# cvjena/semantic-embeddings

Measured on AMD Instinct MI355X. Metric: retrieval_Mpairs_per_sec, higher is better.
Workload: dtype f32

## Files before the change

semantic-embeddings_amd/csrc/rank_rows.hip:

```cpp
#include "se_common.h"
#include <stdlib.h>
#include <atomic>
#include <type_traits>

namespace se {

constexpr int RK_THREADS = 512;
constexpr int RK_WAVES = RK_THREADS / WAVE;
constexpr int RK_ITEMS = 16;
constexpr int RK_TILE = RK_THREADS * RK_ITEMS;
constexpr int RK_WCHUNK = RK_TILE / RK_WAVES;
constexpr int RK_NB = 256;

struct RankLds {
    uint32_t gbase[4][RK_NB];
    uint32_t wcnt[RK_WAVES][RK_NB];
    uint32_t tile_start[RK_NB];
    uint32_t wave_tot[RK_WAVES];
    uint32_t tkeys[RK_TILE];
    uint32_t tidx[RK_TILE];
};

__device__ __forceinline__ uint32_t wave_excl_scan(uint32_t v, uint32_t &total)
{
// ... 11 lines not shown
    RankLds &L = *reinterpret_cast<RankLds *>(rk_raw);
    const int tid = threadIdx.x, lane = tid & 63, wave = tid >> 6;
    const uint64_t lt_mask = (lane == 0) ? 0ull : (~0ull >> (64 - lane));

    uint32_t *kA = ws + (int64_t)blockIdx.x * 4 * n_pad;
    uint32_t *iA = kA + n_pad, *kB = iA + n_pad, *iB = kB + n_pad;
    const int ntiles = (N + RK_TILE - 1) / RK_TILE;

    for (int64_t row = blockIdx.x; row < Q; row += gridDim.x) {
        const float *drow = pdist + row * ldp;

        wg_barrier();
        for (int i = tid; i < 4 * RK_NB; i += RK_THREADS) (&L.gbase[0][0])[i] = 0;
        wg_barrier();
        for (int i = tid; i < N; i += RK_THREADS) {
            const uint32_t key = canon_key(drow[i]);
            atomicAdd(&L.gbase[0][key & 0xFF], 1u);
            atomicAdd(&L.gbase[1][(key >> 8) & 0xFF], 1u);
            atomicAdd(&L.gbase[2][(key >> 16) & 0xFF], 1u);
            atomicAdd(&L.gbase[3][key >> 24], 1u);
        }
        wg_barrier();
        if (wave < 4) {
            uint32_t c[4], s = 0;
#pragma unroll
            for (int j = 0; j < 4; j++) { c[j] = L.gbase[wave][lane * 4 + j]; s += c[j]; }
            uint32_t tot;
            uint32_t run = wave_excl_scan(s, tot);
#pragma unroll
            for (int j = 0; j < 4; j++) { L.gbase[wave][lane * 4 + j] = run; run += c[j]; }
        }
        wg_barrier();

#pragma unroll 1
        for (int p = 0; p < 4; p++) {
            const int shift = p * 8;
            const uint32_t *sk = (p & 1) ? kA : kB;
            const uint32_t *si = (p & 1) ? iA : iB;
            uint32_t *dk = (p & 1) ? kB : kA;
            uint32_t *di = (p & 1) ? iB : iA;
            const bool last = (p == 3);
#pragma unroll 1
            for (int t = 0; t < ntiles; t++) {
                const int tbase = t * RK_TILE;
                const int tcount = (N - tbase < RK_TILE) ? (N - tbase) : RK_TILE;
                const int wbeg = wave * RK_WCHUNK;

                uint32_t key[RK_ITEMS], idx[RK_ITEMS];
                if (p == 0) {
#pragma unroll
                    for (int s = 0; s < RK_ITEMS; s++) {
                        const int li = wbeg + s * WAVE + lane;
                        const int gi = tbase + li;
                        const float f = drow[gi < N ? gi : N - 1];
                        key[s] = (li < tcount) ? canon_key(f) : 0xFFFFFFFFu;
                        idx[s] = (uint32_t)gi;
                    }
                } else {
#pragma unroll
                    for (int s = 0; s < RK_ITEMS; s++) {
                        const int li = wbeg + s * WAVE + lane;
                        const int gi = tbase + li;
                        const int gc = gi < N ? gi : N - 1;
                        const uint32_t k = sk[gc], i2 = si[gc];
                        key[s] = (li < tcount) ? k : 0xFFFFFFFFu;
                        idx[s] = i2;
                    }
                }
#pragma unroll
                for (int j = 0; j < RK_NB / WAVE; j++) L.wcnt[wave][j * WAVE + lane] = 0;
#pragma unroll
                for (int s = 0; s < RK_ITEMS; s++) {
                    const int li = wbeg + s * WAVE + lane;
                    if (li < tcount) atomicAdd(&L.wcnt[wave][(key[s] >> shift) & 0xFF], 1u);
                }
                wg_barrier();
                uint32_t my_total = 0;
                if (tid < RK_NB) {
                    uint32_t run = 0;
#pragma unroll
                    for (int w = 0; w < RK_WAVES; w++) {
                        const uint32_t c = L.wcnt[w][tid];
                        L.wcnt[w][tid] = run;
                        run += c;
                    }
                    my_total = run;
                    uint32_t wtot;
                    const uint32_t ex = wave_excl_scan(my_total, wtot);
                    if (lane == 63) L.wave_tot[wave] = wtot;
                    L.tile_start[tid] = ex;
                }
                wg_barrier();
                if (tid < RK_NB) {
                    uint32_t add = 0;
                    for (int w = 0; w < wave; w++) add += L.wave_tot[w];
                    const uint32_t st = L.tile_start[tid] + add;
                    L.tile_start[tid] = st;
#pragma unroll
                    for (int w = 0; w < RK_WAVES; w++) L.wcnt[w][tid] += st;
                }
                wg_barrier();

                volatile uint32_t *cur = L.wcnt[wave];
#pragma unroll
                for (int s = 0; s < RK_ITEMS; s++) {
                    const int li = wbeg + s * WAVE + lane;
                    const bool valid = li < tcount;
                    const uint32_t dgt = (key[s] >> shift) & 0xFF;
                    uint64_t peers = __ballot(valid);
#pragma unroll
                    for (int bb = 0; bb < 8; bb++) {
                        const bool bit = (dgt >> bb) & 1u;
                        const uint64_t m = __ballot(bit && valid);
                        peers &= bit ? m : ~m;
                    }
                    if (valid) {
                        const int rnk = __popcll(peers & lt_mask);
                        const int npeers = __popcll(peers);
                        const uint32_t base = cur[dgt];
                        if (rnk == npeers - 1) cur[dgt] = base + (uint32_t)npeers;
                        L.tkeys[base + rnk] = key[s];
                        L.tidx[base + rnk] = idx[s];
                    }
                }
                wg_barrier();

#pragma unroll
                for (int j = 0; j < RK_ITEMS; j++) {
                    const int i = j * RK_THREADS + tid;
                    if (i < tcount) {
                        const uint32_t k = L.tkeys[i];
                        const uint32_t id = L.tidx[i];
                        const uint32_t d = (k >> shift) & 0xFF;
                        const uint32_t gpos = L.gbase[p][d] + ((uint32_t)i - L.tile_start[d]);
                        if (last) {
                            if (IDX64) ((int64_t *)rank)[row * ldr + gpos] = (int64_t)id;
                            else ((int32_t *)rank)[row * ldr + gpos] = (int32_t)id;
                        } else {
                            dk[gpos] = k;
                            di[gpos] = id;
                        }
                    }
                }
                wg_barrier();
                if (tid < RK_NB) L.gbase[p][tid] += my_total;
            }
        }
    }
}


constexpr int RR_THREADS = 512;
constexpr int RR_WAVES = RR_THREADS / WAVE;
constexpr int RR_SCAN_THREADS = 512;
constexpr int RR_SCAN_WAVES = RR_SCAN_THREADS / WAVE;
static_assert((53248 + RR_THREADS - 1) / RR_THREADS <= 104, "rows of up to 53,248 columns: 104 keys per thread");
constexpr int RR_G = 8;
constexpr int RR_MAX_N = 53248;

__device__ __forceinline__ void differ_mask(uint32_t d, uint32_t &lo, uint32_t &hi)
{
    lo = 0;
    hi = 0;
#pragma unroll
    for (int bb = 0; bb < 8; bb += 2) {
        uint32_t s0 = (uint32_t)__builtin_amdgcn_sbfe((int)d, bb, 1);
        uint32_t s1 = (uint32_t)__builtin_amdgcn_sbfe((int)d, bb + 1, 1);
        asm volatile("" : "+v"(s0), "+v"(s1));
        const uint64_t m0 = __ballot(s0 != 0), m1 = __ballot(s1 != 0);
        lo = __builtin_amdgcn_bitop3_b32(lo, (uint32_t)m0, s0, 0xF6);
        hi = __builtin_amdgcn_bitop3_b32(hi, (uint32_t)(m0 >> 32), s0, 0xF6);
        lo = __builtin_amdgcn_bitop3_b32(lo, (uint32_t)m1, s1, 0xF6);
        hi = __builtin_amdgcn_bitop3_b32(hi, (uint32_t)(m1 >> 32), s1, 0xF6);
    }
}

constexpr uint32_t RR_KEY_NAN = 0xFF900000u;
__device__ __forceinline__ uint32_t rr_pad_key(uint32_t lane) { return 0xFFA00000u + ((lane % 6u) << 20) + (lane << 11) + lane; }
__device__ __forceinline__ uint32_t rr_key(uint32_t u, bool pad, uint32_t pad_key)
{
    const uint32_t sx = (uint32_t)((int32_t)u >> 31);
    uint32_t k = __builtin_amdgcn_bitop3_b32(u, sx, 0x80000000u, 0x1E);
    k -= sx;
    const float f = __uint_as_float(u);
    k = (f != f) ? RR_KEY_NAN : k;
    return pad ? pad_key : k;
}

__device__ __forceinline__ int32_t rr_clamp_i32(int32_t x, int32_t lo, int32_t hi) { return min(max(x, lo), hi); }

template <typename T>
__device__ __forceinline__ void opaque(T &x) { asm volatile("" : "+v"(x)); }

__device__ __forceinline__ uint32_t lds_off(const void *p) { return (uint32_t)(uintptr_t)p; }
__device__ __forceinline__ void lds_wait() { asm volatile("s_waitcnt lgkmcnt(0)" ::: "memory"); }
__device__ __forceinline__ void lds_st16_lo(uint32_t addr, uint32_t v) { asm volatile("ds_write_b16 %0, %1" ::"v"(addr), "v"(v) : "memory"); }
__device__ __forceinline__ void lds_st16_hi(uint32_t addr, uint32_t v) { asm volatile("ds_write_b16_d16_hi %0, %1" ::"v"(addr), "v"(v) : "memory"); }
__device__ __forceinline__ uint32_t rr_dst_mad(uint32_t ir, uint32_t xb)
{
    uint32_t a;
    asm("v_mad_u32_u16 %0, %1, 2, %2" : "=v"(a) : "v"(ir), "s"(xb));
    return a;
}
template <int OFF>
__device__ __forceinline__ void lds_ld16(uint32_t &dst, uint32_t addr) { asm volatile("ds_read_u16 %0, %1 offset:%2" : "=v"(dst) : "v"(addr), "n"(OFF) : "memory"); }
template <int OFF>
__device__ __forceinline__ void lds_ld16x4_tr(uint64_t &dst, uint32_t addr) { asm volatile("ds_read_b64_tr_b16 %0, %1 offset:%2" : "=v"(dst) : "v"(addr), "n"(OFF) : "memory"); }
template <int K, typename T>
__device__ __forceinline__ void lds_wait_le(T &landed) { asm volatile("s_waitcnt lgkmcnt(%1)" : "+v"(landed) : "n"(K) : "memory"); }

constexpr int RR_RING = 12;
__host__ __device__ constexpr uint32_t rr_tr_lane_off(uint32_t lane) { return 128u * ((lane >> 2) & 3u) + 32u * (lane >> 4) + 8u * (lane & 3u); }
template <int ITEMS, bool HI, int I = 0>
struct RRRead {
    static constexpr int NT = ITEMS / 4, OPS = NT + ITEMS % 4, D = RR_RING / 2 - 1;
    static constexpr uint32_t SEL_LO16 = HI ? 0x05040100u : 0x03020504u;
    static constexpr uint32_t SEL_HI16 = HI ? 0x07060100u : 0x03020706u;
    static __device__ __forceinline__ void run(uint32_t (&a)[ITEMS], uint64_t (&t)[RR_RING / 2], uint32_t (&u)[4], uint32_t rt, uint32_t rb)
    {
        if constexpr (I < NT) lds_ld16x4_tr<I * 4 * WAVE * 2>(t[I % (RR_RING / 2)], rt);
        else if constexpr (I < OPS) lds_ld16<(3 * NT + I) * WAVE * 2>(u[I - NT], rb);
        if constexpr (I >= D) {
            constexpr int J = I - D;
            constexpr int newest = (I < OPS ? I : OPS - 1);
            if constexpr (J < NT) {
                uint64_t &v = t[J % (RR_RING / 2)];
                lds_wait_le<newest - J>(v);
                const uint32_t lo = (uint32_t)v, hi = (uint32_t)(v >> 32);
                a[4 * J + 0] = __builtin_amdgcn_perm(lo, a[4 * J + 0], SEL_LO16);
                a[4 * J + 1] = __builtin_amdgcn_perm(lo, a[4 * J + 1], SEL_HI16);
                a[4 * J + 2] = __builtin_amdgcn_perm(hi, a[4 * J + 2], SEL_LO16);
                a[4 * J + 3] = __builtin_amdgcn_perm(hi, a[4 * J + 3], SEL_HI16);
            } else {
                lds_wait_le<newest - J>(u[J - NT]);
                a[3 * NT + J] = __builtin_amdgcn_perm(u[J - NT], a[3 * NT + J], SEL_LO16);
            }
        }
        if constexpr (I + 1 < OPS + D) RRRead<ITEMS, HI, I + 1>::run(a, t, u, rt, rb);
    }
};
template <int ITEMS, bool HI>
__device__ __forceinline__ void rr_read_back(uint32_t (&a)[ITEMS], uint64_t (&ring)[RR_RING / 2], uint32_t rt, uint32_t rb)
{
    uint32_t u[4];
    RRRead<ITEMS, HI>::run(a, ring, u, rt, rb);
}

template <int ITEMS, int V, int S0, int I = 0>
struct RRRankFinish {
    static __device__ __forceinline__ void run(uint32_t (&ir)[ITEMS], uint32_t (&key)[ITEMS], uint32_t (&rnk)[V], uint32_t (&base)[V])
    {
        lds_wait_le<2 * (V - 1 - I) + 1>(base[I]);
        ir[S0 + I] = (ir[S0 + I] & 0xFFFF0000u) | (base[I] + rnk[I]);
        opaque(ir[S0 + I]);
        opaque(key[S0 + I]);
        if constexpr (I + 1 < V) RRRankFinish<ITEMS, V, S0, I + 1>::run(ir, key, rnk, base);
    }
};

template <int ITEMS, int S0 = 0>
struct RRRank {
    static __device__ __forceinline__ void run(uint32_t (&ir)[ITEMS], uint32_t (&key)[ITEMS], int shift, int lane, uint32_t cb)
    {
        constexpr int V = (ITEMS - S0 < RR_G) ? (ITEMS - S0) : RR_G;
        static_assert(2 * V - 1 <= 15, "lgkmcnt counts to 15");
        uint32_t rnk[V], base[V];
#pragma unroll
        for (int g = 0; g < V; g++) {
            const uint32_t d = (key[S0 + g] >> shift) & 0xFFu;
            uint32_t dlo, dhi;
            differ_mask(d, dlo, dhi);
            rnk[g] = (uint32_t)lane - wave_prefix_count(dlo, dhi);
            const uint32_t ca = cb + (d << 2);
            asm volatile("ds_read_b32 %0, %1" : "=v"(base[g]) : "v"(ca) : "memory");
            if (rnk[g] == 0) {
                const uint32_t np = 64u - (uint32_t)(__popc(dlo) + __popc(dhi));
                asm volatile("ds_add_u32 %0, %1" ::"v"(ca), "v"(np) : "memory");
            }
        }
        RRRankFinish<ITEMS, V, S0>::run(ir, key, rnk, base);
        __builtin_amdgcn_sched_barrier(0);
        if constexpr (S0 + V < ITEMS) RRRank<ITEMS, S0 + V>::run(ir, key, shift, lane, cb);
    }
};

typedef int rr_i32x4 __attribute__((ext_vector_type(4)));
typedef long long rr_i64x2 __attribute__((ext_vector_type(2)));
constexpr int RR_GH = 8;
constexpr int RR_HW_BITS = 11;
constexpr int RR_WIDE_WORDS = 2048;
constexpr uint32_t RR_TWO_SPAN = (1u << 24) - 3u;
constexpr int RR_TWO_OUT = 256;
constexpr int RR_IMG_RUN = 8;
constexpr int RR_IMG_WL = 3072;
constexpr int RR_IMG_MAX_ITEMS = 98;
constexpr uint32_t RR_IMG_NAN_PADHI = 0xFF0u;
constexpr int RR_IMG_SET_WORDS = 2048;
template <int ITEMS, bool PEEL, int S = 0>
struct RRRankHW {
    static __device__ __forceinline__ void run(uint32_t (&ir)[ITEMS], uint32_t (&key)[ITEMS], uint32_t (&r)[RR_GH], uint32_t (&sh)[RR_GH],
                                               uint32_t (&grp)[RR_GH], uint32_t shift, uint32_t hshift, uint32_t wlo, uint32_t whi, uint32_t cb,
                                               int lane, bool peel)
    {
        constexpr int SLOT = S % RR_GH;
        uint32_t ca = 0, inc = 0, shv = 0, g = 0xFFFFFFFFu;
        uint64_t part = ~0ull;
        if constexpr (S < ITEMS) {
            const uint32_t w = __builtin_amdgcn_ubfe(key[S], shift, wlo);
            const uint32_t h = __builtin_amdgcn_ubfe(key[S], hshift, whi);
            ca = cb + (w << 2);
            if constexpr (PEEL) {
                shv = h << 4;
                inc = 1u << shv;
            } else {
                inc = __umul24(h, 0xFFFFu) + 1u;
                shv = __umul24(h, 0x0202u) + 0x07060100u;
            }
            if constexpr (PEEL) {
                if (peel) {
                    const uint32_t d = w | (h << 11);
                    const bool in = (d == (uint32_t)__builtin_amdgcn_readfirstlane((int)d));
                    const uint64_t m = __ballot(in);
                    if (in) g = wave_prefix_count(m);
                    if (lane == 0) inc = (uint32_t)__popcll(m) << shv;
                    part = ~m | 1ull;
                }
            }
        }
        if constexpr (S >= RR_GH) {
            constexpr int J = S - RR_GH;
            constexpr int younger = ((S < ITEMS ? S : ITEMS) - 1) - J;
            lds_wait_le<younger>(r[SLOT]);
            if constexpr (PEEL) {
                const uint32_t lead = (uint32_t)__builtin_amdgcn_readfirstlane((int)r[SLOT]);
                const uint32_t own = (grp[SLOT] != 0xFFFFFFFFu) ? lead : r[SLOT];
                const uint32_t rank = __builtin_amdgcn_ubfe(own, sh[SLOT], 16u) + (grp[SLOT] != 0xFFFFFFFFu ? grp[SLOT] : 0u);
                ir[J] = (ir[J] & 0xFFFF0000u) | rank;
            } else {
                ir[J] = __builtin_amdgcn_perm(ir[J], r[SLOT], sh[SLOT]);
            }
            opaque(ir[J]);
            opaque(key[J]);
        }
        if constexpr (S < ITEMS) {
            sh[SLOT] = shv;
            grp[SLOT] = g;
            if constexpr (PEEL) {
                uint64_t saved;
                r[SLOT] = 0;
                asm volatile("s_and_saveexec_b64 %0, %4\n\tds_add_rtn_u32 %1, %2, %3\n\ts_mov_b64 exec, %0"
                             : "=&s"(saved), "+v"(r[SLOT])
                             : "v"(ca), "v"(inc), "s"(part)
                             : "memory");
            } else {
                asm volatile("ds_add_rtn_u32 %0, %1, %2" : "=v"(r[SLOT]) : "v"(ca), "v"(inc) : "memory");
            }
        }
        __builtin_amdgcn_sched_barrier(0);
        if constexpr (S + 1 < ITEMS + RR_GH) RRRankHW<ITEMS, PEEL, S + 1>::run(ir, key, r, sh, grp, shift, hshift, wlo, whi, cb, lane, peel);
    }
};

// ... 192 lines not shown
            }
            RR_T(8)
        }
        if constexpr (WIDE && VAR == 2) {
            uint32_t *stat = wave_tot;
            uint2 *outl = reinterpret_cast<uint2 *>(wcnt);
            const int n_row = row_len(row);
            int32_t mxi = 0;
            uint32_t umx = 0;
#pragma unroll
            for (int s = 0; s + 1 < ITEMS; s += 2) {
                mxi = max(max(mxi, rr_clamp_i32((int32_t)key[s], 0, 0x7F800000)), rr_clamp_i32((int32_t)key[s + 1], 0, 0x7F800000));
                umx = max(max(umx, key[s]), key[s + 1]);
            }
            if constexpr (ITEMS & 1) { mxi = max(mxi, rr_clamp_i32((int32_t)key[ITEMS - 1], 0, 0x7F800000)); umx = max(umx, key[ITEMS - 1]); }
            mxi = umx > 0xFF800000u ? 0x7F800000 : mxi;
#pragma unroll
            for (int off = 32; off > 0; off >>= 1) mxi = max(mxi, __shfl_xor(mxi, off, 64));
            if (lane == 0) stat[wave] = (uint32_t)mxi;
            if (tid == 0) stat[2 * RR_WAVES] = 0;
            RR_T(9)
            wg_barrier();
            RR_T(10)
#pragma unroll
            for (int w = 0; w < RR_WAVES; w++) mxi = max(mxi, (int32_t)stat[w]);
            const int32_t kmax = __builtin_amdgcn_readfirstlane(mxi);
            const int32_t lo = kmax > (int32_t)RR_TWO_SPAN ? kmax - (int32_t)RR_TWO_SPAN : 1, lo1 = lo - 1;
            uint32_t below_l = 0;
            {
                int wpos = wpos0;
                opaque(wpos);
#pragma unroll
                for (int s = 0; s < ITEMS; s++) below_l += ((int32_t)key[s] < lo) ? 1u : 0u;
                if (wave_s * (ITEMS * WAVE) + ITEMS * WAVE > n_row) {
                    int32_t lo_b = lo;
                    opaque(lo_b);
                    RR_PAD_LOOP(n_row, below_l -= (wpos + s * WAVE >= n_row && (int32_t)key[s] < lo_b) ? 1u : 0u;)
                }
            }
            uint32_t below_w = below_l;
#pragma unroll
            for (int off = 32; off > 0; off >>= 1) below_w += (uint32_t)__shfl_xor((int)below_w, off, 64);
            if (lane == 0) stat[RR_WAVES + wave] = below_w;
            RR_T(11)
            wg_barrier();
            uint32_t below = 0;
#pragma unroll
            for (int w = 0; w < RR_WAVES; w++) below += stat[RR_WAVES + w];
            two = kmax > 0 && below <= (uint32_t)RR_TWO_OUT;
            n_out = (int)below;
            if (two) {
                int wpos = wpos0;
                opaque(wpos);
                if (below_w != 0) {
                    int32_t lo_c = lo;
                    opaque(lo_c);
#pragma unroll
                    for (int s = 0; s < ITEMS; s++)
                        if ((int32_t)key[s] < lo_c && wpos + s * WAVE < n_row)
                            outl[atomicAdd(&stat[2 * RR_WAVES], 1u)] = make_uint2(rr_key(key[s], false, 0u), (uint32_t)(wpos + s * WAVE));
                }
#pragma unroll
                for (int s = 0; s < ITEMS; s++)
                    key[s] = (uint32_t)rr_clamp_i32(__builtin_elementwise_sub_sat((int32_t)key[s], lo1), 0, 0xFFFFFF) << 8;
                if (wave_s * (ITEMS * WAVE) + ITEMS * WAVE > n_row) {
                    RR_PAD_LOOP(n_row, key[s] = (wpos + s * WAVE >= n_row) ? 0xFFFFFF00u : key[s];)
                }
            } else {
                RR_CANON(n_row)
            }
            RR_T(8)
        }
        __builtin_amdgcn_sched_barrier(0);
        {
            int wpos = wpos0;
            opaque(wpos);
#pragma unroll
            for (int s = 0; s < ITEMS; s++) ir[s] = (uint32_t)(wpos + s * WAVE) << 16;
        }
#pragma unroll 1
        for (int p = 0; p < NPASS; p++) {
            const int shift = two ? 8 + 12 * p : (WIDE ? p * 10 : p * BITS);
            const int end = two ? (p == 1 ? 32 : 20)
                                : (WIDE ? (p == 2 ? 32 : shift + 10) : ((shift + BITS < 32) ? shift + BITS : 32));
            const bool wide = WIDE && (two || p == 2);
            uint32_t *pcnt = wcnt;
            int pcw = CNT_WORDS;
            const bool shared0 = IMG && two && p == 0;
            if (shared0) {
                pcnt = wlist;
                pcw = 0;
            } else if (wide) {
                if (!(RAWKEYS && two && p == 0)) wg_barrier();
                pcnt = reinterpret_cast<uint32_t *>(xbuf);
                pcw = RR_WIDE_WORDS;
            }
            uint32_t *mycnt = pcnt + wave * pcw;
            const uint32_t cb = lds_off(mycnt);
            auto one_set = [&]() -> bool {
                if constexpr (!IMG) return false;
                int z = pcw;
                asm volatile("" : "+s"(z));
                return z == 0;
            };
            if constexpr (IMG) {
                if (!one_set()) {
#pragma unroll
                    for (int j = 0; j < CNT_WORDS / (4 * WAVE); j++) reinterpret_cast<uint4 *>(mycnt)[j * WAVE + lane] = make_uint4(0u, 0u, 0u, 0u);
                    if (wide) {
#pragma unroll
                        for (int j = CNT_WORDS / (4 * WAVE); j < RR_WIDE_WORDS / (4 * WAVE); j++) reinterpret_cast<uint4 *>(mycnt)[j * WAVE + lane] = make_uint4(0u, 0u, 0u, 0u);
                    }
                }
            } else {
#pragma unroll
                for (int j = 0; j < CNT_WORDS / WAVE; j++) mycnt[j * WAVE + lane] = 0;
                if (wide) {
#pragma unroll
                    for (int j = CNT_WORDS / WAVE; j < RR_WIDE_WORDS / WAVE; j++) mycnt[j * WAVE + lane] = 0;
                }
            }
            [[maybe_unused]] const uint32_t wlo = wide ? 11u : 10u, whi = (uint32_t)(end - shift) - wlo, hshift = (uint32_t)(shift + (int)wlo) & 31u;
            if constexpr (HWORD) {
                if (wave_live) {
                    uint32_t hr[RR_GH], hs[RR_GH], hg[RR_GH];
                    RRRankHW<ITEMS, PEEL>::run(ir, key, hr, hs, hg, (uint32_t)shift, hshift, wlo, whi, cb, lane, end >= 32 && !two);
                }
            }
            else RRRank<ITEMS>::run(ir, key, shift, lane, cb);
            lds_wait();
            RR_T(1)
            wg_barrier();
            if constexpr (!HWORD) {
            uint32_t ex = 0;
            if (tid < RK_NB) {
                uint32_t run = 0;
#pragma unroll
                for (int w = 0; w < RR_WAVES; w++) run += wcnt[w * RK_NB + tid];
                uint32_t wtot;
                ex = wave_excl_scan(run, wtot);
                if (lane == 63) wave_tot[wave] = wtot;
            }
            wg_barrier();
            if (tid < RK_NB) {
                for (int w = 0; w < wave; w++) ex += wave_tot[w];
#pragma unroll
                for (int w = 0; w < RR_WAVES; w++) {
                    const uint32_t c = wcnt[w * RK_NB + tid];
                    wcnt[w * RK_NB + tid] = ex;
                    ex += c;
                }
            }
            } else {
                const bool scanner = tid < RR_SCAN_THREADS;
                const int st = scanner ? tid : 0;
                uint32_t T0 = 0, T1 = 0, U0 = 0, U1 = 0;
#pragma unroll
                for (int w = 0; w < RR_WAVES; w++) {
                    if (w == 1 && one_set()) break;
                    const uint2 v = *reinterpret_cast<const uint2 *>(pcnt + w * pcw + 2 * st);
                    T0 += v.x; T1 += v.y;
                }
                if (wide) {
                    __builtin_amdgcn_sched_barrier(0);
#pragma unroll
                    for (int w = 0; w < RR_WAVES; w++) {
                        if (w == 1 && one_set()) break;
                        const uint2 v = *reinterpret_cast<const uint2 *>(pcnt + w * pcw + CNT_WORDS + 2 * st);
                        U0 += v.x; U1 += v.y;
                    }
                    __builtin_amdgcn_sched_barrier(0);
                }
                uint32_t wtot, wtot2 = 0, ex2 = 0;
                uint32_t ex = wave_excl_scan(T0 + T1, wtot);
                if (wide) ex2 = wave_excl_scan(U0 + U1, wtot2);
                if (scanner && lane == 63) { wave_tot[wave] = wtot; wave_tot[RR_SCAN_WAVES + wave] = wtot2; }
                wg_barrier();
                uint32_t all = 0, all2 = 0;
#pragma unroll
                for (int w = 0; w < RR_SCAN_WAVES; w++) {
                    const uint32_t wt = wave_tot[w], wt2 = wave_tot[RR_SCAN_WAVES + w];
                    all += wt; all2 += wt2;
                    ex += (w < wave) ? wt : 0u;
                    ex2 += (w < wave) ? wt2 : 0u;
                }
                ex2 += all;
                const uint32_t hi = (all + all2) << 16;
                ex += hi; ex2 += hi;
                if (scanner) {
                uint32_t s0 = ex, s1 = ex + T0;
#pragma unroll
                for (int w = 0; w < RR_WAVES; w++) {
                    if (w == 1 && one_set()) break;
                    uint2 *wp = reinterpret_cast<uint2 *>(pcnt + w * pcw + 2 * tid);
                    const uint2 v = *wp;
                    *wp = make_uint2(s0, s1);
                    s0 += v.x; s1 += v.y;
                }
                if (wide) {
                    __builtin_amdgcn_sched_barrier(0);
                    s0 = ex2; s1 = ex2 + U0;
#pragma unroll
                    for (int w = 0; w < RR_WAVES; w++) {
                        if (w == 1 && one_set()) break;
                        uint2 *wp = reinterpret_cast<uint2 *>(pcnt + w * pcw + CNT_WORDS + 2 * tid);
                        const uint2 v = *wp;
                        *wp = make_uint2(s0, s1);
                        s0 += v.x; s1 += v.y;
                    }
                }
                }
            }
            wg_barrier();
            RR_T(2)
            if (!(IMG && two)) { RR_PREFETCH_NEXT_ROW() }
            if (wave_live) {
#pragma unroll
            for (int s0 = 0; s0 < ITEMS; s0 += 8) {
                uint32_t first[8];
#pragma unroll
                for (int g = 0; g < 8; g++)
                    if (s0 + g < ITEMS) {
                        if constexpr (HWORD) first[g] = reinterpret_cast<const uint16_t *>(mycnt)[(__builtin_amdgcn_ubfe(key[s0 + g], (uint32_t)shift, wlo) << 1) | __builtin_amdgcn_ubfe(key[s0 + g], hshift, whi)];
                        else first[g] = mycnt[(key[s0 + g] >> shift) & 0xFFu];
                    }
#pragma unroll
                for (int g = 0; g < 8; g++)
                    if (s0 + g < ITEMS) {
                        ir[s0 + g] += first[g];
                        opaque(ir[s0 + g]);
                    }
                __builtin_amdgcn_sched_barrier(0);
            }
            }
            if (wide && !one_set()) wg_barrier();
            RR_T(3)
            if constexpr (LOAD_IN_SCATTER) {
                if (end >= 32) break;
            }
            if (wave_live) {
                if constexpr (LOAD_IN_SCATTER) {
                    RR_IDX_SCATTER_IMG()
                } else {
#pragma unroll
                    for (int s = 0; s < ITEMS; s++) { opaque(ir[s]); lds_st16_hi(RR_DST(ir[s]), ir[s]); }
                }
            }
            lds_wait();
            wg_barrier();
            RR_T(4)
            const bool last = end >= 32;
            if (last) {
                if constexpr (!SEG) break;
                else {
                    RR_STREAM_PLANE(0, row)
                    wg_barrier();
                }
            } else {
                if (wave_live) rr_read_back<ITEMS, true>(ir, ring, rt, rb);
                lds_wait();
                wg_barrier();
            }
            RR_T(5)
            if (wave_live) {
#pragma unroll
                for (int s = 0; s < ITEMS; s++) { opaque(ir[s]); lds_st16_hi(RR_DST(ir[s]), key[s]); }
            }
            lds_wait();
            wg_barrier();
            if (SEG && last) {
                RR_STREAM_PLANE(1, row)
            } else {
                if (wave_live) rr_read_back<ITEMS, true>(key, ring, rt, rb);
                lds_wait();
            }
            if (end < 16 || SEG) {
                wg_barrier();
                if (wave_live) {
#pragma unroll
                    for (int s = 0; s < ITEMS; s++) { opaque(ir[s]); lds_st16_lo(RR_DST(ir[s]), key[s]); }
                }
                lds_wait();
                wg_barrier();
                if (SEG && last) break;
                if (wave_live) rr_read_back<ITEMS, false>(key, ring, rt, rb);
                lds_wait();
            }
            RR_T(6)
        }
#undef RR_DST
        if constexpr (WIDE && VAR == 2) {
            if (two && n_out > 1) {
                const uint2 *outl = reinterpret_cast<const uint2 *>(wcnt);
                if (tid < n_out) {
                    const uint2 me = outl[tid];
                    int r = 0;
                    for (int j = 0; j < n_out; j++) {
                        const uint2 o = outl[j];
                        r += (o.x < me.x || (o.x == me.x && o.y < me.y)) ? 1 : 0;
                    }
                    xbuf[r] = (uint16_t)me.y;
                }
                wg_barrier();
            }
        }
        [[maybe_unused]] bool img_fail = false;
        if constexpr (IMG) {
            const float *drow = row_ptr(more ? row + gridDim.x : row);
            int wpos = wpos0;
            opaque(wpos);
            if constexpr (LOAD_IN_SCATTER) {
                RR_IDX_SCATTER_IMG(RR_LOAD_ONE(drow, wpos, s, n_next))
                lds_wait();
                wg_barrier();
                RR_T(4)
            } else {
#pragma unroll
                for (int s = 0; s < ITEMS; s++) RR_LOAD_ONE(drow, wpos, s, n_next)
            }
        }
        if constexpr (IMG) {
            if (two) {
                int n_row = row_len(row);
                int tsc = wave_s * WAVE + (int)wave_prefix_count(~0u, ~0u);
                opaque(n_row);
                opaque(tsc);
                const float *drow_cur = row_ptr(row);
                constexpr int NS = RR_THREADS * ITEMS;
                constexpr int NG = (NS / 8 + RR_THREADS - 1) / RR_THREADS;
                uint32_t S[NG];
                uint32_t nstart = 0;
                uint4 xg[NG];
                uint32_t nxg[NG];
#pragma unroll
                for (int g = 0; g < NG; g++) {
                    const int b0 = (tsc + RR_THREADS * g) * 8;
                    const int bs = b0 < NS ? b0 : 0;
                    xg[g] = *reinterpret_cast<const uint4 *>(xbuf + bs);
                    nxg[g] = xbuf[(tsc & 63) == 63 ? (bs + 8 < NS ? bs + 8 : bs) : 0];
                }
                constexpr int TD = 1;
                uint32_t t[TD + 1][9];
                auto tag_reads = [&](int g, uint32_t (&tt)[9]) {
                    const uint32_t xi[4] = {xg[g].x, xg[g].y, xg[g].z, xg[g].w};
#pragma unroll
                    for (int j = 0; j < 4; j++) {
                        tt[2 * j] = tagb[xi[j] & 0xFFFFu];
                        tt[2 * j + 1] = tagb[xi[j] >> 16];
                    }
                    tt[8] = tagb[nxg[g]];
                };
#pragma unroll
                for (int g = 0; g < TD && g < NG; g++) tag_reads(g, t[g % (TD + 1)]);
#pragma unroll
                for (int g = 0; g < NG; g++) {
                    if (g + TD < NG) tag_reads(g + TD, t[(g + TD) % (TD + 1)]);
                    const uint32_t (&tc)[9] = t[g % (TD + 1)];
                    const bool live = (tsc + RR_THREADS * g) * 8 < n_row - 1;
                    const uint32_t A = tc[0] | (tc[1] << 8) | (tc[2] << 16) | (tc[3] << 24), B = tc[4] | (tc[5] << 8) | (tc[6] << 16) | (tc[7] << 24);
                    const uint32_t t8 = (uint32_t)__builtin_amdgcn_update_dpp((int)tc[8], (int)tc[0], 0x130, 0xF, 0xF, false);
                    const uint32_t zA = A ^ __builtin_amdgcn_alignbyte(B, A, 1), zB = B ^ __builtin_amdgcn_alignbyte(t8, B, 1);
                    const uint32_t uA = (zA & 0x7F7F7F7Fu) + 0x7F7F7F7Fu, uB = (zB & 0x7F7F7F7Fu) + 0x7F7F7F7Fu;
                    const uint32_t eA = __builtin_amdgcn_bitop3_b32(uA, zA, 0x80808080u, 0x02), eB = __builtin_amdgcn_bitop3_b32(uB, zB, 0x80808080u, 0x02);
                    S[g] = live ? ((eA >> 7) | (eB >> 3)) : 0u;
                    nstart += (uint32_t)__popc(S[g]);
                }
                uint32_t slot = 0;
                {
                    const uint32_t ca = lds_off(&ictl[0]);
                    asm volatile("ds_add_rtn_u32 %0, %1, %2\n\ts_waitcnt lgkmcnt(0)" : "=v"(slot) : "v"(ca), "v"(nstart) : "memory");
                }
#pragma unroll
                for (int g = 0; g < NG; g++) {
                    uint32_t st = S[g];
                    const int b0 = (tsc + RR_THREADS * g) * 8;
                    while (st) {
                        const int bit = __builtin_ctz(st);
                        st &= st - 1u;
                        const int pos = b0 + (bit & 4) + (bit >> 3);
                        if (slot < (uint32_t)RR_IMG_WL) wlist[slot] = pos < n_row - 1 ? (uint32_t)pos : 0xFFFFFFFFu;
                        slot++;
                    }
                }
                if constexpr (PROF) { RR_T(9) }
                wg_barrier();
                const uint32_t nwork = ictl[0];
                img_fail = nwork > (uint32_t)RR_IMG_WL;
                RR_T(11)
                if (!img_fail) {
                    constexpr int GB = 2;
#pragma unroll 1
                    for (uint32_t e0 = 0; e0 < nwork; e0 += RR_THREADS * GB) {
                        uint32_t pp[GB], im[GB], ia[GB], ib[GB], ic[GB], id[GB], tm[GB], t0[GB], t2[GB], t3[GB], ka[GB], kb[GB], kc[GB];
#pragma unroll
                        for (int k = 0; k < GB; k++) {
                            const uint32_t e = e0 + (uint32_t)(k * RR_THREADS + tsc);
                            pp[k] = e < nwork ? wlist[e] : 0xFFFFFFFFu;
                        }
#pragma unroll
                        for (int k = 0; k < GB; k++) {
                            const uint32_t p = pp[k] != 0xFFFFFFFFu ? pp[k] : 0u;
                            im[k] = xbuf[p ? p - 1u : 0u]; ia[k] = xbuf[p]; ib[k] = xbuf[p + 1];
                            ic[k] = xbuf[p + 2 < (uint32_t)NS ? p + 2 : p]; id[k] = xbuf[p + 3 < (uint32_t)NS ? p + 3 : p];
                        }
#pragma unroll
                        for (int k = 0; k < GB; k++) { tm[k] = tagb[im[k]]; t0[k] = tagb[ia[k]]; t2[k] = tagb[ic[k]]; t3[k] = tagb[id[k]]; }
#pragma unroll
                        for (int k = 0; k < GB; k++) {
                            const bool mine = pp[k] != 0xFFFFFFFFu && !(pp[k] != 0u && tm[k] == t0[k]);
                            const bool three = mine && (int)pp[k] + 2 < n_row && t2[k] == t0[k];
                            ka[k] = kb[k] = kc[k] = 0u;
                            if (mine) {
                                ka[k] = __float_as_uint(drow_cur[ia[k]]);
                                kb[k] = __float_as_uint(drow_cur[ib[k]]);
                            }
                            if (three) kc[k] = __float_as_uint(drow_cur[ic[k]]);
                        }
                        uint32_t rare = 0;
#pragma unroll
                        for (int k = 0; k < GB; k++) {
                            if (pp[k] == 0xFFFFFFFFu) continue;
                            const uint32_t p = pp[k];
                            if (p != 0u && tm[k] == t0[k]) continue;
                            const bool three = (int)p + 2 < n_row && t2[k] == t0[k];
                            const bool more4 = three && (int)p + 3 < n_row && t3[k] == t0[k];
                            const uint64_t ca = ((uint64_t)rr_key(ka[k], false, 0u) << 32) | ia[k], cb = ((uint64_t)rr_key(kb[k], false, 0u) << 32) | ib[k],
                                           cc = ((uint64_t)rr_key(kc[k], false, 0u) << 32) | ic[k];
                            if (!three) {
                                if (ca > cb) { xbuf[p] = (uint16_t)ib[k]; xbuf[p + 1] = (uint16_t)ia[k]; }
                            } else if (!more4) {
                                const uint32_t ab = ca < cb, ac = ca < cc, bc = cb < cc;
                                const uint32_t ra = 2u - ab - ac, rb = ab + 1u - bc, rc = ac + bc;
                                if (ra != 0u || rb != 1u) {
                                    xbuf[p + ra] = (uint16_t)ia[k]; xbuf[p + rb] = (uint16_t)ib[k]; xbuf[p + rc] = (uint16_t)ic[k];
                                }
                            } else rare |= 1u << k;
                        }
                        static_assert(GB == 2, "the entry is picked by one select");
#pragma unroll 1
                        for (uint32_t k = 0; k < (uint32_t)GB; k++) {
                            if (!((rare >> k) & 1u)) continue;
                            const uint32_t p = k ? pp[1] : pp[0], tg = k ? t0[1] : t0[0];
                            int len = 4;
                            while (len <= RR_IMG_RUN && (int)p + len < n_row && tagb[xbuf[p + len]] == tg) len++;
                            if (len > RR_IMG_RUN) { ictl[1] = 1u; continue; }
                            uint32_t idx[RR_IMG_RUN];
                            uint64_t kk[RR_IMG_RUN];
#pragma unroll
                            for (int j = 0; j < RR_IMG_RUN; j++) idx[j] = xbuf[p + (uint32_t)(j < len ? j : 0)];
#pragma unroll
                            for (int j = 0; j < RR_IMG_RUN; j++) kk[j] = ((uint64_t)rr_key(__float_as_uint(drow_cur[idx[j]]), false, 0u) << 32) | idx[j];
#pragma unroll
                            for (int j = 0; j < RR_IMG_RUN; j++) {
                                uint32_t r = 0;
#pragma unroll
                                for (int i = 0; i < RR_IMG_RUN; i++)
                                    if (i != j) r += (i < len && kk[i] < kk[j]) ? 1u : 0u;
                                if (j < len) xbuf[p + r] = (uint16_t)idx[j];
                            }
                        }
                    }
                    wg_barrier();
                    img_fail = ictl[1] != 0u;
                }
                RR_T(10)
            }
        }
        if (!IMG || img_fail) {
            const float *drow = row_ptr((IMG && img_fail) ? row : (more ? row + gridDim.x : row));
            int wpos = wpos0;
            opaque(wpos);
#pragma unroll
            for (int s = 0; s < ITEMS; s++) RR_LOAD_ONE(drow, wpos, s, n_next)
        }
        if constexpr (IMG) {
#pragma unroll
            for (int s = 0; s < ITEMS; s++) opaque(key[s]);
            asm volatile("s_waitcnt vmcnt(0)" : "+v"(pf_sink) : : "memory");
        }
        int wt = tid;
        opaque(wt);
        const bool write_out = !IMG || !img_fail;
        if constexpr (SEG) {
            RR_STREAM_PLANE(2, row)
        } else if (!write_out) {
        } else if (idx64 == 2) {
            uint16_t *o = (uint16_t *)rank + row * ldr;
            _Pragma("unroll 2") for (int j = wt * 8; j < N; j += RR_THREADS * 8) {
                if (vec_ok && j + 7 < N) {
                    const rr_i32x4 v = *reinterpret_cast<const rr_i32x4 *>(xbuf + j);
                    __builtin_nontemporal_store(v, reinterpret_cast<rr_i32x4 *>(o + j));
                } else {
                    for (int e = 0; e < 8 && j + e < N; e++) o[j + e] = xbuf[j + e];
                }
            }
        } else if (idx64) {
            int64_t *o = (int64_t *)rank + row * ldr;
            uint2 nv = *reinterpret_cast<const uint2 *>(xbuf + (wt * 4 < N ? wt * 4 : 0));
            _Pragma("unroll 1") for (int j = wt * 4; j < N; j += RR_THREADS * 4) {
                const uint2 v = nv;
                const int jn = j + RR_THREADS * 4;
                nv = *reinterpret_cast<const uint2 *>(xbuf + (jn < N ? jn : 0));
                const int64_t e0 = v.x & 0xFFFFu, e1 = v.x >> 16, e2 = v.y & 0xFFFFu, e3 = v.y >> 16;
                if (vec_ok && j + 3 < N) {
                    __builtin_nontemporal_store((rr_i64x2){e0, e1}, reinterpret_cast<rr_i64x2 *>(o + j));
                    __builtin_nontemporal_store((rr_i64x2){e2, e3}, reinterpret_cast<rr_i64x2 *>(o + j + 2));
                } else {
                    o[j] = e0;
                    if (j + 1 < N) o[j + 1] = e1;
                    if (j + 2 < N) o[j + 2] = e2;
                    if (j + 3 < N) o[j + 3] = e3;
                }
            }
        } else {
            int32_t *o = (int32_t *)rank + row * ldr;
            constexpr int RR_WO = 4;
            _Pragma("unroll 1") for (int j0 = wt * 4; j0 < N; j0 += RR_THREADS * 4 * RR_WO) {
                uint2 v[RR_WO];
#pragma unroll
                for (int u = 0; u < RR_WO; u++) {
                    const int j = j0 + u * RR_THREADS * 4;
                    v[u] = *reinterpret_cast<const uint2 *>(xbuf + (j < N ? j : 0));
                }
#pragma unroll
                for (int u = 0; u < RR_WO; u++) {
                    const int j = j0 + u * RR_THREADS * 4;
                    if (j >= N) break;
                    const int e0 = v[u].x & 0xFFFFu, e1 = v[u].x >> 16, e2 = v[u].y & 0xFFFFu, e3 = v[u].y >> 16;
// ... 841 lines not shown
```

Measured before the change: 242,700.

## Vectorize count-scan with b128 LDS ops and make run-start detection wave-local

Rewrites the digit-count prefix scan so each scanner thread handles four counters via 128-bit LDS reads and writes, with a compile-time per-stride recursion that pipelines loads and stores. The separate wide/narrow scans are merged into a single pass. The run-start tagging in the image path now assigns contiguous chunks per wave and gets the neighbour tag via readfirstlane/DPP instead of an extra xbuf/tagb gather per thread. The scatter address computation also switches to an explicit v_mad_u32_u16. These changes aim to cut LDS instruction count and a scattered gather, but they rely on layout assumptions that are more complex to verify.

```diff
diff --git a/semantic-embeddings_amd/csrc/rank_rows.hip b/semantic-embeddings_amd/csrc/rank_rows.hip
--- a/semantic-embeddings_amd/csrc/rank_rows.hip
+++ b/semantic-embeddings_amd/csrc/rank_rows.hip
@@ -187,8 +187,6 @@
 
 constexpr int RR_THREADS = 512;
 constexpr int RR_WAVES = RR_THREADS / WAVE;
-constexpr int RR_SCAN_THREADS = 512;
-constexpr int RR_SCAN_WAVES = RR_SCAN_THREADS / WAVE;
 static_assert((53248 + RR_THREADS - 1) / RR_THREADS <= 104, "rows of up to 53,248 columns: 104 keys per thread");
 constexpr int RR_G = 8;
 constexpr int RR_MAX_N = 53248;
@@ -243,6 +241,26 @@
 __device__ __forceinline__ void lds_ld16x4_tr(uint64_t &dst, uint32_t addr) { asm volatile("ds_read_b64_tr_b16 %0, %1 offset:%2" : "=v"(dst) : "v"(addr), "n"(OFF) : "memory"); }
 template <int K, typename T>
 __device__ __forceinline__ void lds_wait_le(T &landed) { asm volatile("s_waitcnt lgkmcnt(%1)" : "+v"(landed) : "n"(K) : "memory"); }
+
+typedef uint32_t rr_u32x4 __attribute__((ext_vector_type(4)));
+template <int OFF>
+__device__ __forceinline__ void lds_ld128(rr_u32x4 &dst, uint32_t addr) { asm volatile("ds_read_b128 %0, %1 offset:%2" : "=v"(dst) : "v"(addr), "n"(OFF) : "memory"); }
+template <int OFF>
+__device__ __forceinline__ void lds_st128(uint32_t addr, rr_u32x4 v) { asm volatile("ds_write_b128 %0, %1 offset:%2" ::"v"(addr), "v"(v), "n"(OFF) : "memory"); }
+template <int STRIDE_BYTES, int TRIPS, int W = 0>
+struct RRScanBases {
+    static_assert((TRIPS - 1) * STRIDE_BYTES < 65536, "immediate offsets");
+    static __device__ __forceinline__ void run(uint32_t a, rr_u32x4 &s, rr_u32x4 (&v)[2])
+    {
+        if constexpr (W == 0) lds_ld128<0>(v[0], a);
+        if constexpr (W + 1 < TRIPS) lds_ld128<(W + 1) * STRIDE_BYTES>(v[(W + 1) & 1], a);
+        lds_wait_le<(W > 0 ? 1 : 0) + (W + 1 < TRIPS ? 1 : 0)>(v[W & 1]);
+        lds_st128<W * STRIDE_BYTES>(a, s);
+        s += v[W & 1];
+        opaque(s);
+        if constexpr (W + 1 < TRIPS) RRScanBases<STRIDE_BYTES, TRIPS, W + 1>::run(a, s, v);
+    }
+};
 
 constexpr int RR_RING = 12;
 __host__ __device__ constexpr uint32_t rr_tr_lane_off(uint32_t lane) { return 128u * ((lane >> 2) & 3u) + 32u * (lane >> 4) + 8u * (lane & 3u); }
@@ -741,64 +759,47 @@
                 }
             }
             } else {
-                const bool scanner = tid < RR_SCAN_THREADS;
-                const int st = scanner ? tid : 0;
-                uint32_t T0 = 0, T1 = 0, U0 = 0, U1 = 0;
-#pragma unroll
-                for (int w = 0; w < RR_WAVES; w++) {
-                    if (w == 1 && one_set()) break;
-                    const uint2 v = *reinterpret_cast<const uint2 *>(pcnt + w * pcw + 2 * st);
-                    T0 += v.x; T1 += v.y;
-                }
-                if (wide) {
-                    __builtin_amdgcn_sched_barrier(0);
+                const bool scanner = wave_s < (wide ? RR_WIDE_WORDS : CNT_WORDS) / (4 * WAVE);
+                uint4 *const my4 = reinterpret_cast<uint4 *>(pcnt + 4 * tid);
+                auto per_stride = [&](auto &&loop) {
+                    if constexpr (IMG) {
+                        if (one_set()) { loop(std::integral_constant<int, 0>(), std::integral_constant<int, 1>()); return; }
+                    }
+                    if constexpr (WIDE) {
+                        if (wide) { loop(std::integral_constant<int, RR_WIDE_WORDS>(), std::integral_constant<int, RR_WAVES>()); return; }
+                    }
+                    loop(std::integral_constant<int, CNT_WORDS>(), std::integral_constant<int, RR_WAVES>());
+                };
+                uint32_t T0 = 0, T1 = 0, T2 = 0, T3 = 0;
+                if (scanner)
+                    per_stride([&](auto STRIDE, auto TRIPS) {
+#pragma unroll
+                        for (int w = 0; w < decltype(TRIPS)::value; w++) {
+                            const uint4 v = my4[w * (decltype(STRIDE)::value / 4)];
+                            T0 += v.x; T1 += v.y; T2 += v.z; T3 += v.w;
+                            if (w % 4 == 3) __builtin_amdgcn_sched_barrier(0);
+                        }
+                    });
+                uint32_t wtot;
+                uint32_t ex = wave_excl_scan(T0 + T1 + T2 + T3, wtot);
+                if (lane == 63) wave_tot[wave] = wtot;
+                wg_barrier();
+                {
+                    const uint4 wa = *reinterpret_cast<const uint4 *>(wave_tot), wb = *reinterpret_cast<const uint4 *>(wave_tot + 4);
+                    const uint32_t wt[RR_WAVES] = {wa.x, wa.y, wa.z, wa.w, wb.x, wb.y, wb.z, wb.w};
+                    uint32_t all = 0;
 #pragma unroll
                     for (int w = 0; w < RR_WAVES; w++) {
-                        if (w == 1 && one_set()) break;
-                        const uint2 v = *reinterpret_cast<const uint2 *>(pcnt + w * pcw + CNT_WORDS + 2 * st);
-                        U0 += v.x; U1 += v.y;
+                        all += wt[w];
+                        ex += (w < wave_s) ? wt[w] : 0u;
                     }
-                    __builtin_amdgcn_sched_barrier(0);
-                }
-                uint32_t wtot, wtot2 = 0, ex2 = 0;
-                uint32_t ex = wave_excl_scan(T0 + T1, wtot);
-                if (wide) ex2 = wave_excl_scan(U0 + U1, wtot2);
-                if (scanner && lane == 63) { wave_tot[wave] = wtot; wave_tot[RR_SCAN_WAVES + wave] = wtot2; }
-                wg_barrier();
-                uint32_t all = 0, all2 = 0;
-#pragma unroll
-                for (int w = 0; w < RR_SCAN_WAVES; w++) {
-                    const uint32_t wt = wave_tot[w], wt2 = wave_tot[RR_SCAN_WAVES + w];
-                    all += wt; all2 += wt2;
-                    ex += (w < wave) ? wt : 0u;
-                    ex2 += (w < wave) ? wt2 : 0u;
-                }
-                ex2 += all;
-                const uint32_t hi = (all + all2) << 16;
-                ex += hi; ex2 += hi;
-                if (scanner) {
-                uint32_t s0 = ex, s1 = ex + T0;
-#pragma unroll
-                for (int w = 0; w < RR_WAVES; w++) {
-                    if (w == 1 && one_set()) break;
-                    uint2 *wp = reinterpret_cast<uint2 *>(pcnt + w * pcw + 2 * tid);
-                    const uint2 v = *wp;
-                    *wp = make_uint2(s0, s1);
-                    s0 += v.x; s1 += v.y;
-                }
-                if (wide) {
-                    __builtin_amdgcn_sched_barrier(0);
-                    s0 = ex2; s1 = ex2 + U0;
-#pragma unroll
-                    for (int w = 0; w < RR_WAVES; w++) {
-                        if (w == 1 && one_set()) break;
-                        uint2 *wp = reinterpret_cast<uint2 *>(pcnt + w * pcw + CNT_WORDS + 2 * tid);
-                        const uint2 v = *wp;
-                        *wp = make_uint2(s0, s1);
-                        s0 += v.x; s1 += v.y;
-                    }
-                }
-                }
+                    ex += all << 16;
+                }
+                if (scanner)
+                    per_stride([&](auto STRIDE, auto TRIPS) {
+                        rr_u32x4 sb = {ex, ex + T0, ex + T0 + T1, ex + T0 + T1 + T2}, v2[2];
+                        RRScanBases<decltype(STRIDE)::value * 4, decltype(TRIPS)::value>::run(lds_off(my4), sb, v2);
+                    });
             }
             wg_barrier();
             RR_T(2)
@@ -853,7 +854,7 @@
             RR_T(5)
             if (wave_live) {
 #pragma unroll
-                for (int s = 0; s < ITEMS; s++) { opaque(ir[s]); lds_st16_hi(RR_DST(ir[s]), key[s]); }
+                for (int s = 0; s < ITEMS; s++) { opaque(ir[s]); lds_st16_hi(rr_dst_mad(ir[s], xb), key[s]); }
             }
             lds_wait();
             wg_barrier();
@@ -867,7 +868,7 @@
                 wg_barrier();
                 if (wave_live) {
 #pragma unroll
-                    for (int s = 0; s < ITEMS; s++) { opaque(ir[s]); lds_st16_lo(RR_DST(ir[s]), key[s]); }
+                    for (int s = 0; s < ITEMS; s++) { opaque(ir[s]); lds_st16_lo(rr_dst_mad(ir[s], xb), key[s]); }
                 }
                 lds_wait();
                 wg_barrier();
@@ -916,38 +917,45 @@
                 opaque(tsc);
                 const float *drow_cur = row_ptr(row);
                 constexpr int NS = RR_THREADS * ITEMS;
-                constexpr int NG = (NS / 8 + RR_THREADS - 1) / RR_THREADS;
+                constexpr int GW = WAVE * ITEMS / 8;
+                constexpr int NG = (GW + WAVE - 1) / WAVE;
+                constexpr bool FULL_LAST = GW % WAVE == 0;
+                int gsc = wave_s * GW + (tsc & 63);
+                opaque(gsc);
                 uint32_t S[NG];
                 uint32_t nstart = 0;
                 uint4 xg[NG];
-                uint32_t nxg[NG];
 #pragma unroll
                 for (int g = 0; g < NG; g++) {
-                    const int b0 = (tsc + RR_THREADS * g) * 8;
+                    const int b0 = (gsc + WAVE * g) * 8;
                     const int bs = b0 < NS ? b0 : 0;
                     xg[g] = *reinterpret_cast<const uint4 *>(xbuf + bs);
-                    nxg[g] = xbuf[(tsc & 63) == 63 ? (bs + 8 < NS ? bs + 8 : bs) : 0];
-                }
+                }
+                [[maybe_unused]] uint32_t edge = 0;
+                if constexpr (FULL_LAST) edge = tagb[xbuf[wave_s + 1 < RR_WAVES ? (wave_s + 1) * (ITEMS * WAVE) : 0]];
                 constexpr int TD = 1;
-                uint32_t t[TD + 1][9];
-                auto tag_reads = [&](int g, uint32_t (&tt)[9]) {
+                uint32_t t[TD + 1][8];
+                auto tag_reads = [&](int g, uint32_t (&tt)[8]) {
                     const uint32_t xi[4] = {xg[g].x, xg[g].y, xg[g].z, xg[g].w};
 #pragma unroll
                     for (int j = 0; j < 4; j++) {
                         tt[2 * j] = tagb[xi[j] & 0xFFFFu];
                         tt[2 * j + 1] = tagb[xi[j] >> 16];
                     }
-                    tt[8] = tagb[nxg[g]];
                 };
 #pragma unroll
                 for (int g = 0; g < TD && g < NG; g++) tag_reads(g, t[g % (TD + 1)]);
 #pragma unroll
                 for (int g = 0; g < NG; g++) {
                     if (g + TD < NG) tag_reads(g + TD, t[(g + TD) % (TD + 1)]);
-                    const uint32_t (&tc)[9] = t[g % (TD + 1)];
-                    const bool live = (tsc + RR_THREADS * g) * 8 < n_row - 1;
+                    const uint32_t (&tc)[8] = t[g % (TD + 1)];
+                    bool live = (gsc + WAVE * g) * 8 < n_row - 1;
+                    if (!FULL_LAST && g == NG - 1) live = live && (tsc & 63) < GW % WAVE;
                     const uint32_t A = tc[0] | (tc[1] << 8) | (tc[2] << 16) | (tc[3] << 24), B = tc[4] | (tc[5] << 8) | (tc[6] << 16) | (tc[7] << 24);
-                    const uint32_t t8 = (uint32_t)__builtin_amdgcn_update_dpp((int)tc[8], (int)tc[0], 0x130, 0xF, 0xF, false);
+                    uint32_t nx0 = tc[0];
+                    if (g + 1 < NG) nx0 = (uint32_t)__builtin_amdgcn_readfirstlane((int)t[(g + 1) % (TD + 1)][0]);
+                    else if constexpr (FULL_LAST) nx0 = edge;
+                    const uint32_t t8 = (uint32_t)__builtin_amdgcn_update_dpp((int)nx0, (int)tc[0], 0x130, 0xF, 0xF, false);
                     const uint32_t zA = A ^ __builtin_amdgcn_alignbyte(B, A, 1), zB = B ^ __builtin_amdgcn_alignbyte(t8, B, 1);
                     const uint32_t uA = (zA & 0x7F7F7F7Fu) + 0x7F7F7F7Fu, uB = (zB & 0x7F7F7F7Fu) + 0x7F7F7F7Fu;
                     const uint32_t eA = __builtin_amdgcn_bitop3_b32(uA, zA, 0x80808080u, 0x02), eB = __builtin_amdgcn_bitop3_b32(uB, zB, 0x80808080u, 0x02);
@@ -962,7 +970,7 @@
 #pragma unroll
                 for (int g = 0; g < NG; g++) {
                     uint32_t st = S[g];
-                    const int b0 = (tsc + RR_THREADS * g) * 8;
+                    const int b0 = (gsc + WAVE * g) * 8;
                     while (st) {
                         const int bit = __builtin_ctz(st);
                         st &= st - 1u;
```

Measured after the change: 243,800 (median of 6 runs). No clear change (+0.4%).
